# artbataev/end2end

Hardware: AMD Instinct MI355X
Metric: ctc_fwd_bwd_frames_per_sec (higher is better)
Workload: dtype f32; 1 GPU; ctc_fwd_bwd_B256_T1000_V29_S200_f32; B_per_gpu=256, T=1000, V=29, S_max=200, input=raw logits (log-softmax fused)

## Files before the change

### end2end_amd/csrc/ctc_loss_fast_h1.hip

```cpp
#include "fast_common.h"

namespace e2e {
namespace fastk {
namespace {

constexpr int kHxNP = 2;
constexpr int kHxHalo = 8;
constexpr int kHxOwnLanes = 64 - kHxHalo;
constexpr int kHxProducers = 2;
constexpr int kHxOwn = kHxNP * kHxOwnLanes;
constexpr int kHxMaxW = 4 / kHxNP;
constexpr int kHxWaves = 2 * kHxMaxW + 2 + 2 * kHxProducers + 2;

struct HxLds {
  static constexpr int kCkPad = 4;
  static constexpr int kCkCells = 2 * 4 * kHxOwnLanes + 2 * kCkPad;
  int ring;
  int blk_bytes;
  int filled;
  int sortcnt;
  int bnd;
  int bw;
  int dump;
  int zacc;
  int prog;
  int exw;
  int mxl;
  int ckb;
  int ckdone;
  int total;
  __host__ __device__ HxLds(int V) {
    bw = 4;
    ring = 0;
    blk_bytes = ((V + 1) * kRow + 16) * 8;
    filled = ring + 2 * kRingBlks * blk_bytes;
    sortcnt = filled + 2 * kRingBlks * 4;
    bnd = (sortcnt + 130 * 4 + 15) & ~15;
    dump = bnd + 2 * bw * kHaloSlots * kHxHalo * 32;
    zacc = dump + 12288;
    prog = zacc + 64;
    exw = prog + 2 * 8 * 4;
    mxl = exw + 2 * kHaloSlots * 4;
    ckb = mxl + 2 * kHaloSlots * 4 * 64 * 4;
    ckdone = ckb + 2 * 2 * kCkCells * 8;
    total = ckdone + 16;
  }
};

#ifdef E2E_FAST_PROFILE
#define HX_TL(k) { if (w == 0 && lane == 0 && b < 256) { unsigned long long* g = g_tl + ((size_t)b * 2 + DIR) * 12 + 2 * (k); \
    g[0] = __builtin_amdgcn_s_memtime(); g[1] = wall_clock64(); } }
#else
#define HX_TL(k)
#endif
template <int DIR>
__device__ __forceinline__ void hx_chain_wave(const FastParams& p, int b, int T, int S, unsigned char* smem, const HxLds hl,
                                              int lane, int w, int W) {
  lds_u8* L0 = (lds_u8*)smem;
  HX_TL(1)
  const int V = p.V, blank = p.blank, L = 2 * S + 1;
  const int nblk = (T + kBlk - 1) / kBlk;
  const int M = (T - 1) >> 3;
  const int ring_off = hl.ring + DIR * kRingBlks * hl.blk_bytes;
  volatile int* myfilled = reinterpret_cast<int*>(smem + hl.filled) + DIR * kRingBlks;
  __builtin_amdgcn_s_setprio(3);
  unsigned long long prof_fill = 0, prof_nb = 0, prof_lag = 0, prof_t0 = __builtin_amdgcn_s_memtime();
  (void)prof_fill; (void)prof_nb; (void)prof_lag; (void)prof_t0;

  const int g0 = kHxOwn * w + kHxNP * (DIR == 0 ? lane - kHxHalo : lane);
  const bool halo = DIR == 0 ? lane < kHxHalo : lane >= kHxOwnLanes;
  const bool edge = DIR == 0 ? lane >= 64 - kHxHalo : lane < kHxHalo;
  const int up = DIR == 0 ? (w > 0 ? w - 1 : 7) : w + 1;
  const int64_t* tg = p.targets + (int64_t)b * p.tgt_stride;
  const float r_tilt = fast_tilt(S, T);
  const double rr2 = (double)r_tilt * (double)r_tilt, inv_rr = 1.0 / (double)r_tilt;
  const double skip_w = (double)(r_tilt * r_tilt);
  int lab[kHxNP]; double sk[kHxNP];
  bool badlab = false;
#pragma unroll
  for (int r = 0; r < kHxNP; r++) {
    const int gi = g0 + r, li = DIR == 0 ? gi : gi - 1;
    const bool lin = li >= 0 && li < S;
    const int lv = lin ? label_of(tg[li]) : -1;
    lab[r] = (lin && lv >= 0 && lv < V) ? lv : V;
    if (DIR == 0) {
      const int lpv = (li >= 1 && li - 1 < S) ? label_of(tg[li - 1]) : -1;
      sk[r] = (lin && li >= 1 && lv != blank && lpv != lv) ? skip_w : 0.0;
      badlab |= !halo && lin && (lv == blank || lv < 0 || lv >= V);
    } else {
      const int tj = (gi >= 1 && gi < S) ? label_of(tg[gi]) : -1;
      sk[r] = (gi >= 1 && gi < S && lv != blank && tj != lv) ? skip_w : 0.0;
    }
  }
  if (DIR == 0 && __any(badlab)) { if (lane == 0) atomicOr(&p.flags[b], 2); }
  const bool cond = (T > 1 || L == 1);

  const int a_sync = hl.prog;
  const int o_prog = DIR * 32, o_exw = hl.exw - hl.prog + DIR * (kHaloSlots * 4), o_ckdone = hl.ckdone - hl.prog + 4 * DIR;
  const int a_mxl = hl.mxl + ((DIR * kHaloSlots * 4 + w) * 64 + lane) * 4;
  const int up_rec = DIR == 0 ? (w > 0 ? w - 1 : hl.bw - 1) : w + 1;
  const int a_bnd_up = hl.bnd + ((DIR * hl.bw + up_rec) * kHaloSlots * kHxHalo + (lane & (kHxHalo - 1))) * 32;
  const int a_bnd_my = edge ? hl.bnd + ((DIR * hl.bw + w) * kHaloSlots * kHxHalo + (lane & (kHxHalo - 1))) * 32
                            : hl.dump + lane * 32;
  const int a_ck = halo ? hl.dump + 4096 + lane * 32
                        : hl.ckb + (DIR * 2 * HxLds::kCkCells + HxLds::kCkPad) * 8 + (DIR == 0 ? 16 * g0 : 16 * g0 - 8);
  int a_lab[kHxNP];
#pragma unroll
  for (int r = 0; r < kHxNP; r++) a_lab[r] = ring_off + lab[r] * (kRow * 8);
  const int a_yw = ring_off + (V + 1) * (kRow * 8);

  double Bc[kHxNP], Lc[kHxNP];
#pragma unroll
  for (int r = 0; r < kHxNP; r++) { Bc[r] = 0.0; Lc[r] = 0.0; }
  double yb_prev = 0.0, wb_prev = 0.0;
  int e_total = 0;
  int nck = 0, ckbuf = 0;
  int lead = 0;
  auto need_blocks = [&](int k) {
    if (lead < k) {
      PROF_SPIN_BEGIN
      for (;;) {
        int a = peek(&myfilled[0]);
#pragma unroll
        for (int f = 1; f < kHxProducers; f++) a = min(a, peek(&myfilled[f]));
        lead = __builtin_amdgcn_readfirstlane(a);
        if (lead >= k) break;
        __builtin_amdgcn_s_sleep(1);
      }
      asm volatile("" ::: "memory");
      PROF_SPIN_END(prof_fill)
    }
  };

  double e[kHxNP][kBlk], ybw[2 * kBlk];
  auto load_half = [&](int slot_bytes, auto half_tag) {
    constexpr int H = decltype(half_tag)::value;
    lds_u8* py = L0 + (a_yw + slot_bytes);
#pragma unroll
    for (int q = 3; q >= 1; q--) {
      const h_d2 y = *(volatile lds_d2*)(py + 64 * H + 16 * q);
      ybw[8 * H + 2 * q] = y.x; ybw[8 * H + 2 * q + 1] = y.y;
    }
#pragma unroll
    for (int r = 0; r < kHxNP; r++) {
      const h_d2 a = *(volatile lds_d2*)(L0 + (a_lab[r] + slot_bytes) + 32 * H + 16); e[r][4 * H + 2] = a.x; e[r][4 * H + 3] = a.y;
    }
#pragma unroll
    for (int r = 0; r < kHxNP; r++) {
      const h_d2 a = *(volatile lds_d2*)(L0 + (a_lab[r] + slot_bytes) + 32 * H); e[r][4 * H] = a.x; e[r][4 * H + 1] = a.y;
    }
    { const h_d2 y = *(volatile lds_d2*)(py + 64 * H); ybw[8 * H] = y.x; ybw[8 * H + 1] = y.y; }
  };
  auto read_edge = [&](int slot, h_d2 (&hv)[kHxNP]) {
#pragma unroll
    for (int r = 0; r < kHxNP; r++) hv[r] = *(volatile lds_d2*)(L0 + a_bnd_up + slot * 256 + 16 * r);
  };

  int hprog = 0;
  h_d2 hv[kHxNP];
#pragma unroll
  for (int r = 0; r < kHxNP; r++) hv[r] = h_d2{0.0, 0.0};
  int ckd = 0;
  auto run_block = [&](int n, auto steady_tag, auto slot_tag, auto ck_tag) {
    constexpr bool STEADY = decltype(steady_tag)::value;
    constexpr int SLOT = decltype(slot_tag)::value, CK = decltype(ck_tag)::value;
    const int slot = SLOT >= 0 ? SLOT : (n & (kRingBlks - 1));
    const int nslot = SLOT >= 0 ? ((SLOT + 1) & (kRingBlks - 1)) : ((n + 1) & (kRingBlks - 1));
    const int pslot = SLOT >= 0 ? ((SLOT + 7) & (kRingBlks - 1)) : ((n + 7) & (kRingBlks - 1));
    const bool refill = SLOT >= 0 ? (SLOT % kHxNP) == 0 : (n % kHxNP) == 0;
    const bool publish = SLOT >= 0 ? (SLOT % kHxNP) == kHxNP - 1 : (n % kHxNP) == kHxNP - 1;
    load_half(slot * hl.blk_bytes, std::integral_constant<int, 1>{});
    if (refill && (STEADY || n > 0)) {
      if (__builtin_amdgcn_readfirstlane(hprog) < n) {
        PROF_SPIN_BEGIN HALO_WAIT(__builtin_amdgcn_readfirstlane(*(volatile lds_int*)(L0 + a_sync + o_prog + 4 * up)) >= n); PROF_SPIN_END(prof_nb)
        read_edge(pslot, hv);
      }
      if (halo) {
#pragma unroll
        for (int r = 0; r < kHxNP; r++) { Bc[r] = hv[r].x; Lc[r] = hv[r].y; }
      }
    }
    const bool want_next = STEADY ? true : n + 1 < nblk;
    const int tbase = block_time(DIR, n, 0, T);
    int xw = 0;
#pragma unroll
    for (int tt = 0; tt < kBlk; tt++) {
      const int t = DIR == 0 ? tbase + tt : tbase - tt;
      const double yb = ybw[2 * tt], wb = ybw[2 * tt + 1];
      if (tt == 4) {
        xw = *(volatile lds_int*)(L0 + a_sync + o_exw + 4 * slot);
        if (CK != 0) ckd = *(volatile lds_int*)(L0 + a_sync + o_ckdone);
        if (want_next) need_blocks(n + 2);
        load_half(nslot * hl.blk_bytes, std::integral_constant<int, 0>{});
      }
      if (tt == 6 && publish) {
        hprog = *(volatile lds_int*)(L0 + a_sync + o_prog + 4 * up);
        read_edge(slot, hv);
      }
      if (STEADY || t < T) {
        const bool first = !STEADY && (DIR == 0 ? t == 0 : t == T - 1);
        if (first) {
#pragma unroll
          for (int r = 0; r < kHxNP; r++) {
            if (DIR == 0) {
              if (g0 + r == 0) { Bc[r] = cond ? 1.0 : 0.0; Lc[r] = rr2 * e[r][tt]; }
            } else {
              if (g0 + r == S) { if (cond) Bc[r] = 1.0; Lc[r] = rr2 * e[r][tt]; }
            }
          }
        } else if (DIR == 0) {
          double nb = from_prev_lane(Lc[kHxNP - 1]);
#pragma unroll
          for (int r = 0; r < kHxNP; r++) {
            const double ol = Lc[r];
            const double Bn = __builtin_fma(Bc[r], yb_prev, nb);
            double tl = __builtin_fma(Bc[r], wb_prev, ol);
            tl = __builtin_fma(sk[r], nb, tl);
            Lc[r] = tl * e[r][tt]; Bc[r] = Bn; nb = ol;
          }
        } else {
          double nb = from_next_lane(Lc[0]);
#pragma unroll
          for (int r = kHxNP - 1; r >= 0; r--) {
            const double ol = Lc[r];
            const double Bn = __builtin_fma(Bc[r], yb_prev, nb);
            double tl = __builtin_fma(Bc[r], wb_prev, ol);
            tl = __builtin_fma(sk[r], nb, tl);
            Lc[r] = tl * e[r][tt]; Bc[r] = Bn; nb = ol;
          }
        }
        yb_prev = yb; wb_prev = wb;
        if (tt == 7) {
          int top = max(__double2hiint(Bc[0]), __double2hiint(Lc[0]));
#pragma unroll
          for (int r = 1; r < kHxNP; r++) top = max(top, max(__double2hiint(Bc[r]), __double2hiint(Lc[r])));
          *(volatile lds_int*)(L0 + a_mxl + slot * 1024) = top;
          xw = __builtin_amdgcn_readfirstlane(xw);
          if ((xw >> 12) != n) {
            PROF_SPIN_BEGIN
            int spins = 0;
            do {
              __builtin_amdgcn_s_sleep(1);
              xw = __builtin_amdgcn_readfirstlane(*(volatile lds_int*)(L0 + a_sync + o_exw + 4 * slot));
              if (++spins > (1 << 20)) { atomicOr(&p.flags[b], 128); xw = (n << 12) | 2048; }
            } while ((xw >> 12) != n);
            PROF_SPIN_END(prof_lag)
          }
          const int ex = (xw & 0xfff) - 2048;
#pragma unroll
          for (int r = 0; r < kHxNP; r++) { Bc[r] = ldexp(Bc[r], -ex); Lc[r] = ldexp(Lc[r], -ex); }
          e_total += ex;
          const int kk = DIR == 0 ? (t + 1) : t;
          if ((CK >= 0 ? CK == 1 : ((kk & (kSeg - 1)) == 0 && kk > 0 && kk < T))) {
            if (nck >= 2 && __builtin_amdgcn_readfirstlane(ckd) < nck - 1)
              HALO_WAIT(__builtin_amdgcn_readfirstlane(*(volatile lds_int*)(L0 + a_sync + o_ckdone)) >= nck - 1);
            if (nck == 0) ckbuf = (kk / kSeg) & 1;
            nck++;
            lds_u8* dst = L0 + (a_ck + ckbuf * (HxLds::kCkCells * 8));
#pragma unroll
            for (int r = 0; r < kHxNP; r++) {
              const double cb = Bc[r] * yb_prev, cl = Lc[r] * inv_rr;
              if (DIR == 0) { *(volatile lds_f64*)(dst + 16 * r) = cb; *(volatile lds_f64*)(dst + 16 * r + 8) = cl; }
              else { *(volatile lds_f64*)(dst + 16 * r) = cl; *(volatile lds_f64*)(dst + 16 * r + 8) = cb; }
            }
            ckbuf ^= 1;
          }
        }
      }
    }
    if (publish) {
#pragma unroll
      for (int r = 0; r < kHxNP; r++) { h_d2 v; v.x = Bc[r]; v.y = Lc[r]; *(volatile lds_d2*)(L0 + a_bnd_my + slot * 256 + 16 * r) = v; }
    }
    *(volatile lds_int*)(L0 + a_sync + o_prog + 4 * w) = n + 1;
  };
  {
    typedef std::integral_constant<int, -1> Any;
    need_blocks(1);
    HX_TL(2)
    load_half(0, std::integral_constant<int, 0>{});
    const int steady_end = DIR == 0 ? T / kBlk : nblk;
    run_block(0, std::false_type{}, Any{}, Any{});
    int n = 1;
    if (M - 1 >= 16) {
      for (; n < 8; n++) run_block(n, std::true_type{}, Any{}, Any{});
      auto eight = [&](auto par_tag) {
        constexpr int P = decltype(par_tag)::value;
#define HX_BLK(K) run_block(n + K, std::true_type{}, std::integral_constant<int, K>{}, std::integral_constant<int, ((K & 1) == P) ? 1 : 0>{});
        for (; n + 8 <= M; n += 8) { HX_BLK(0) HX_BLK(1) HX_BLK(2) HX_BLK(3) HX_BLK(4) HX_BLK(5) HX_BLK(6) HX_BLK(7) }
#undef HX_BLK
      };
      if (DIR == 0 || (M & 1)) eight(std::integral_constant<int, 1>{});
      else eight(std::integral_constant<int, 0>{});
    }
    for (; n < steady_end - 1; n++) run_block(n, std::true_type{}, Any{}, Any{});
    for (; n < nblk; n++) run_block(n, std::false_type{}, Any{}, Any{});
  }
  HX_TL(3)
#ifdef E2E_FAST_PROFILE
  if (lane == 0 && b < 256) { unsigned long long* g = g_prof3 + ((size_t)b * 16 + DIR * 8 + w) * 4;
    g[0] = __builtin_amdgcn_s_memtime() - prof_t0; g[1] = prof_fill; g[2] = prof_nb; g[3] = prof_lag; }
#endif
  lds_u8* prog = L0 + hl.prog + DIR * 32;
  if (DIR == 0) {
    double z = 0.0;
    if (!halo) {
#pragma unroll
      for (int r = 0; r < kHxNP; r++) {
        if (g0 + r == S) z += Bc[r] * yb_prev;
        if (g0 + r == S - 1) z += Lc[r];
      }
    }
    for (int o = 32; o > 0; o >>= 1) z += __shfl_xor(z, o, 64);
    *(volatile lds_f64*)(L0 + hl.zacc + 8 * w) = z;
    *(volatile lds_int*)(prog + 4 * w) = nblk + 1;
    if (w == 0) {
      HALO_WAIT(__builtin_amdgcn_readfirstlane(lds_min8(prog)) >= nblk + 1);
      if (lane == 0) {
        double zs = 0.0;
        for (int k = 0; k < W; k++) zs += *(volatile lds_f64*)(L0 + hl.zacc + 8 * k);
        const double rr = (double)r_tilt;
        const double lz = log(zs) + (double)e_total * 0.693147180559945309417 - (double)(L - 1) * log(rr);
        p.logz[2 * b] = lz;
        p.zt2[b] = log2(zs) + (double)e_total;
        p.losses[b] = (float)(-lz);
        if (!(zs > 0.0) || !(zs < __builtin_huge_val())) atomicOr(&p.flags[b], 4);
      }
    }
  } else if (w == 0) {
    const double l0 = Lc[kHxNP - 1];
    if (lane == 0) {
      const double z = (cond ? Bc[0] * yb_prev : 0.0) + l0;
      p.logz[2 * b + 1] = log(z) + (double)e_total * 0.693147180559945309417 - (double)(L - 1) * log((double)r_tilt);
    }
  }
  HX_TL(4)
}

template <int NV, int DIR>
__device__ __forceinline__ void hx_prep_wave(const FastParams& p, int b, int T, int first, unsigned char* smem, const HxLds hl,
                                             int lane, double rr2) {
  constexpr int stride = kHxProducers;
  lds_u8* L0 = (lds_u8*)smem;
  const int V = p.V;
  const int nblk = (T + kBlk - 1) / kBlk, M = (T - 1) >> 3;
  const int tt = lane >> 3, l8 = lane & 7;
  const float ninf = -__builtin_huge_valf();
  constexpr int kFull = NV == 2 ? 0 : NV == 12 ? 8 : NV - 2;
  bool live[NV];
#pragma unroll
  for (int k = 0; k < NV; k++) live[k] = k < kFull || l8 + 8 * k < V;
  const bool contig = p.sV == 1;
  const int64_t xl = (int64_t)b * p.sB + (int64_t)l8 * p.sV;
  const int64_t cstep = 8 * p.sV;
  float* yl = p.ytab + ((size_t)b * p.NS * V + l8) * kSeg;
  const int t_first = DIR == 0 ? tt : 8 * M + 7 - tt;
  lds_u8* prog = L0 + hl.prog + DIR * 32;
  const int a_fill = hl.filled + (DIR * kRingBlks + first) * 4;
  const int a_row = hl.ring + DIR * kRingBlks * hl.blk_bytes + (l8 * kRow + tt) * 8;
  const int a_yw = hl.ring + DIR * kRingBlks * hl.blk_bytes + ((V + 1) * kRow + 2 * tt) * 8;
  const int kb = p.blank >> 3;
  const bool blank_lane = l8 == (p.blank & 7);

  auto row_of = [&](int n) { return DIR == 0 ? t_first + 8 * n : t_first - 8 * n; };
  auto load_block = [&](auto f32_tag, int n, float (&out)[NV]) {
    constexpr bool F32IN = decltype(f32_tag)::value;
    const int t = row_of(n);
    const int tc = min(max(t, 0), T - 1);
    const int64_t xr = xl + (int64_t)tc * p.sT;
    int64_t off[NV];
#pragma unroll
    for (int k = 0; k < NV; k++) off[k] = (k < kFull || live[k]) ? (contig ? (int64_t)(8 * k) : k * cstep) : 0;
    if (F32IN) {
      const float* src = reinterpret_cast<const float*>(p.x) + xr;
#pragma unroll
      for (int k = 0; k < NV; k++) out[k] = src[off[k]];
    } else {
      const unsigned short* src = reinterpret_cast<const unsigned short*>(p.x) + xr;
      unsigned short h[NV];
#pragma unroll
      for (int k = 0; k < NV; k++) h[k] = src[off[k]];
      const bool bf = p.xdt == E2E_BF16;
#pragma unroll
      for (int k = 0; k < NV; k++)
        out[k] = bf ? __uint_as_float((unsigned)h[k] << 16) : (float)__builtin_bit_cast(f16_t, h[k]);
    }
  };
  int consumed = 0;
  float lpmin = 0.f;
  auto process = [&](int n, const float (&xraw)[NV]) {
    constexpr bool STEADY = false;
    const int t = row_of(n);
    const bool row_live = t >= 0 && t < T;
    float xv[NV];
#pragma unroll
    for (int k = 0; k < NV; k++) xv[k] = (row_live && (k < kFull || live[k])) ? xraw[k] : ninf;
    if (n >= kRingBlks) {
      while (consumed < n - kRingBlks + 1) {
        consumed = __builtin_amdgcn_readfirstlane(lds_min8(prog));
        if (consumed < n - kRingBlks + 1) __builtin_amdgcn_s_sleep(1);
      }
      asm volatile("" ::: "memory");
    }
    float y[NV];
    if (p.logprobs) {
#pragma unroll
      for (int k = 0; k < NV; k++) {
        y[k] = exp_le0(xv[k]);
        if (DIR == 0) lpmin = fminf(lpmin, xv[k] > ninf ? xv[k] : 0.f);
      }
    } else {
      float m = xv[0];
#pragma unroll
      for (int k = 1; k < NV; k++) m = fmaxf(m, xv[k]);
      m = row8_max(m);
      float ssum = 0.f;
      const float mM = -m * 1.44269504088896340736f;
#pragma unroll
      for (int k = 0; k < NV; k++) {
        const float d = xv[k] - m;
        y[k] = __builtin_amdgcn_exp2f(fmaf(xv[k], 1.44269504088896340736f, mM)); ssum += y[k];
        if (DIR == 0) lpmin = fminf(lpmin, xv[k] > ninf ? d : 0.f);
      }
      ssum = row8_sum(ssum);
      float inv = __builtin_amdgcn_rcpf(ssum);
      inv = fmaf(fmaf(-ssum, inv, 1.0f), inv, inv);
#pragma unroll
      for (int k = 0; k < NV; k++) y[k] *= inv;
    }
    if (!STEADY) {
#pragma unroll
      for (int k = 0; k < NV; k++) y[k] = row_live ? y[k] : 0.f;
    }
    const int sb = (n & (kRingBlks - 1)) * hl.blk_bytes;
    lds_u8* dst = L0 + (a_row + sb);
#pragma unroll
    for (int k = 0; k < NV; k++) {
      if (k < kFull || live[k]) *(volatile lds_f64*)(dst + k * (8 * kRow * 8)) = (double)y[k];
    }
    {
      float ybl = y[0];
#pragma unroll
      for (int k = 1; k < NV; k++) ybl = kb == k ? y[k] : ybl;
      if (blank_lane) { h_d2 yw; yw.x = (double)ybl; yw.y = rr2 * (double)ybl; *(volatile lds_d2*)(L0 + (a_yw + sb)) = yw; }
    }
    if (DIR == 0 && row_live) {
      float* yrow = yl + (size_t)(t >> 4) * V * kSeg + (t & (kSeg - 1));
#pragma unroll
      for (int k = 0; k < NV; k++) {
        if (k < kFull || live[k]) yrow[8 * k * kSeg] = y[k];
      }
    }
    *(volatile lds_int*)(L0 + a_fill) = n + stride;
  };
  auto run = [&](auto f32_tag) {
    float xa[NV], xb[NV], xc[NV];
    load_block(f32_tag, first, xa);
    load_block(f32_tag, first + stride, xb);
    for (int n = first; n < nblk; n += 3 * stride) {
      load_block(f32_tag, n + 2 * stride, xc); process(n, xa);
      load_block(f32_tag, n + 3 * stride, xa); if (n + stride < nblk) process(n + stride, xb);
      load_block(f32_tag, n + 4 * stride, xb); if (n + 2 * stride < nblk) process(n + 2 * stride, xc);
    }
  };
  if (p.xdt == E2E_F32) run(std::true_type{}); else run(std::false_type{});
  { const bool t1 = __any(lpmin < -69.f), t2 = __any(lpmin < -78.f);
    if (DIR == 0 && t1 && lane == 0) atomicOr(&p.flags[b], t2 ? 64 | 256 : 64); }
}

template <int DIR, int F2PPL>
__device__ __forceinline__ void hx_ckpt_wave(const FastParams& p, int b, int T, int S, lds_u8* L0, const HxLds hl, int lane, int npairs) {
  static_assert(F2PPL == 1 || F2PPL == 2 || F2PPL == 4, "groups of up to four lanes (one DPP quad)");
  const int nblk = (T + kBlk - 1) / kBlk;
  const int nres = DIR == 0 ? T / kBlk : nblk;
  const int M = (T - 1) >> 3;
  lds_u8* prog = L0 + hl.prog + DIR * 32;
  float* ck = (DIR == 0 ? p.ckA : p.ckQ) + (size_t)b * p.NS * p.CELLS;
  int done = 0;
  for (int n = 0; n < nres; n++) {
    const int kk = DIR == 0 ? 8 * (n + 1) : 8 * (M - n);
    if (!((kk & (kSeg - 1)) == 0 && kk > 0 && kk < T)) continue;
    HALO_WAIT(__builtin_amdgcn_readfirstlane(lds_min8(prog)) >= n + 1);
    const int slot = kk / kSeg;
    const int base = hl.ckb + ((DIR * 2 + (slot & 1)) * HxLds::kCkCells + HxLds::kCkPad) * 8;
    h_d2 c[4];
#pragma unroll
    for (int q = 0; q < 4; q++) {
      const int i = 64 * q + lane;
      c[q] = h_d2{0.0, 0.0};
      if (64 * q < npairs) c[q] = *(volatile lds_d2*)(L0 + base + 16 * min(i, npairs - 1));
      if (i >= S) c[q].y = 0.0;
      if (i > S) c[q].x = 0.0;
    }
    *(volatile lds_int*)(L0 + hl.ckdone + 4 * DIR) = ++done;
#pragma unroll
    for (int q = 0; q < 4; q++) {
      if (64 * q >= npairs) break;
      const int i = 64 * q + lane;
      int m = max(__double2hiint(c[q].x), __double2hiint(c[q].y));
      if (F2PPL >= 2) m = max(m, dpp_i<0xB1>(0, m));
      if (F2PPL >= 4) m = max(m, dpp_i<0x4E>(0, m));
      const int own = ((m >> 20) & 0x7ff) - 1023;
      const int st = m > 0 ? own : -30000;
      if (i < npairs && (i & ~(F2PPL - 1)) <= S) {
        float2 o;
        o.x = m > 0 ? (float)ldexp(c[q].x, -own) : 0.f; o.y = m > 0 ? (float)ldexp(c[q].y, -own) : 0.f;
        *reinterpret_cast<float2*>(ck + (size_t)slot * p.CELLS + 2 * i) = o;
        short* cke = p.ckE + (((size_t)b * p.NS + slot) * 2 + DIR) * 64;
        if ((i & (F2PPL - 1)) == 0) cke[i / F2PPL] = (short)st;
      }
    }
  }
}

template <int PPL>
__global__ E2E_KERNEL_ALIGN __launch_bounds__(kHxWaves * 64) void ctc_fast_chain_hx_kernel(FastParams p) {
  extern __shared__ __align__(16) unsigned char smem[];
  const int b = blockIdx.x, tid = threadIdx.x, lane = tid & 63, wid = tid >> 6;
  const int V = p.V;
  const HxLds hl(V);
#ifdef E2E_FAST_PROFILE
  if (tid < 128 && lane == 0 && b < 256) { unsigned long long* g = g_tl + ((size_t)b * 2 + (tid >> 6)) * 12; g[0] = __builtin_amdgcn_s_memtime(); g[1] = wall_clock64(); }
#endif

  if (b == 0 && tid < 32) p.ctl[tid] = 0;
  const int64_t Tq = p.x_len[b], Sq = p.t_len[b];
  const bool bad = Tq < 1 || Tq > p.T || Sq < 0 || Sq > p.Smax;
  if (bad) {
    if (tid == 0) { p.flags[b] = 1; p.losses[b] = __builtin_nanf(""); }
    return;
  }
  const int T = (int)Tq, S = (int)Sq;
  const int W = min(S / kHxOwn + 1, kHxMaxW);
  if (tid == 0) p.flags[b] = 0;
  for (int i = tid; i < p.MW; i += blockDim.x) p.segmask[(size_t)b * p.MW + i] = 0u;
  if (tid < 2 * kRingBlks) reinterpret_cast<int*>(smem + hl.filled)[tid] = (tid & (kRingBlks - 1)) < kHxProducers ? (tid & (kRingBlks - 1)) : 0;
  if (tid < 16) reinterpret_cast<int*>(smem + hl.prog)[tid] = (tid & 7) < W ? 0 : kHaloIdle;
  if (tid < 2 * kHaloSlots) reinterpret_cast<int*>(smem + hl.exw)[tid] = (tid & (kHaloSlots - 1)) < kHaloLag ? ((tid & (kHaloSlots - 1)) << 12) | 2048 : -1;
  if (tid < 8) reinterpret_cast<double*>(smem + hl.zacc)[tid] = 0.0;
  if (tid < 2) reinterpret_cast<int*>(smem + hl.ckdone)[tid] = 0;
  for (int i = tid; i < (hl.dump - hl.bnd) / 16; i += blockDim.x) reinterpret_cast<double2*>(smem + hl.bnd)[i] = double2{0.0, 0.0};
  for (int i = tid; i < 2 * kRingBlks * kBlk; i += blockDim.x)
    reinterpret_cast<double*>(smem + hl.ring + (i / kBlk) * hl.blk_bytes)[V * kRow + (i % kBlk)] = 0;
  __syncthreads();

  constexpr int kChains = 2 * kHxMaxW, kFrame = kChains, kProd = kChains + 2, kCkpt = kProd + 2 * kHxProducers;
  const int wave = __builtin_amdgcn_readfirstlane(wid);
  lds_u8* L0 = (lds_u8*)smem;
  if (wave < kChains) {
    const int d = wave & 1, w = wave >> 1;
    if (w >= W) return;
    if (d == 0) hx_chain_wave<0>(p, b, T, S, smem, hl, lane, w, W);
    else hx_chain_wave<1>(p, b, T, S, smem, hl, lane, w, W);
  } else if (wave == kFrame) halo_frame_wave<0, false, kHaloLag, true>(p, b, T, L0, hl.prog, hl.exw, hl.mxl, 4, lane, W, 0);
  else if (wave == kFrame + 1) halo_frame_wave<1, false, kHaloLag, true>(p, b, T, L0, hl.prog, hl.exw, hl.mxl, 4, lane, W, 0);
  else if (wave == kCkpt) hx_ckpt_wave<0, PPL>(p, b, T, S, L0, hl, lane, kHxOwn * W);
  else if (wave == kCkpt + 1) {
    cellinfo_wave<PPL>(p, b, T, S, reinterpret_cast<int*>(smem + hl.sortcnt), lane);
    hx_ckpt_wave<1, PPL>(p, b, T, S, L0, hl, lane, kHxOwn * W);
  } else {
    const int d = (wave - kProd) & 1;
    const int first = (wave - kProd) >> 1;
    const double rr2 = (double)fast_tilt(S, T) * (double)fast_tilt(S, T);
#define HX_PREP(NVV) { if (d == 0) hx_prep_wave<NVV, 0>(p, b, T, first, smem, hl, lane, rr2); else hx_prep_wave<NVV, 1>(p, b, T, first, smem, hl, lane, rr2); }
    if (V <= 16) HX_PREP(2) else if (V <= 32) HX_PREP(4) else if (V <= 48) HX_PREP(6) else if (V <= 64) HX_PREP(8) else HX_PREP(12)
#undef HX_PREP
  }
}

}

bool h1_supported(int V, int Smax, int ppl) {
  return (ppl == 2 || ppl == 4) && Smax + 1 <= 4 * kHxOwnLanes && HxLds(V).total <= 160 * 1024;
}

Chains h1_chains(int ppl, int V) {
  return Chains{ppl == 4 ? &ctc_fast_chain_hx_kernel<4> : &ctc_fast_chain_hx_kernel<2>, kHxWaves * 64, (size_t)HxLds(V).total};
}

}
}

#ifdef E2E_FAST_PROFILE
extern "C" int e2e_debug_fast_timeline_h1(unsigned long long* host) {
  return hipMemcpyFromSymbol(host, HIP_SYMBOL(e2e::fastk::g_tl), sizeof(unsigned long long) * 256 * 2 * 12) == hipSuccess ? 0 : E2E_ERR_HIP;
}
extern "C" int e2e_debug_fast_profile3_h1(unsigned long long* host, int reset) {
  if (reset) { void* ptr; if (hipGetSymbolAddress(&ptr, HIP_SYMBOL(e2e::fastk::g_prof3)) != hipSuccess) return E2E_ERR_HIP;
    return hipMemset(ptr, 0, sizeof(unsigned long long) * 256 * 16 * 4) == hipSuccess ? 0 : E2E_ERR_HIP; }
  return hipMemcpyFromSymbol(host, HIP_SYMBOL(e2e::fastk::g_prof3), sizeof(unsigned long long) * 256 * 16 * 4) == hipSuccess ? 0 : E2E_ERR_HIP;
}
#endif
```

### end2end_amd/csrc/fast_common.h

```cpp
#pragma once
#include <stdlib.h>
#include <type_traits>

#include "common.h"

#pragma clang fp contract(fast)

#define E2E_KERNEL_ALIGN __attribute__((aligned(65536)))

namespace e2e {
namespace fastk {

constexpr int kSeg = kFastSeg;
constexpr int kBlk = 8;
constexpr int kRingBlks = 8;
constexpr int kRow32 = 12;
constexpr int kRow = 10;
constexpr int kMaxSmallV = 96;
constexpr int kMaxBigV = 224;
constexpr int kMaxHugeV = 448;
__host__ __device__ inline int lstart_ints(int V) { return 64 * ((V + 64) >> 6) + 2; }

struct FastParams {
  const void* x; int xdt;
// ... 73 lines not shown
  v += __int_as_float(__builtin_amdgcn_update_dpp(0, __float_as_int(v), 0x111, 0xf, 0xf, true));
  v += __int_as_float(__builtin_amdgcn_update_dpp(0, __float_as_int(v), 0x112, 0xf, 0xf, true));
  v += __int_as_float(__builtin_amdgcn_update_dpp(0, __float_as_int(v), 0x114, 0xf, 0xf, true));
  v += __int_as_float(__builtin_amdgcn_update_dpp(0, __float_as_int(v), 0x118, 0xf, 0xf, true));
  E2E_ROW_BCAST_STEPS("v_add_f32_dpp", v);
  return v;
}
__device__ __forceinline__ void wave_scan8(float (&v)[8]) {
#pragma unroll
  for (int k = 0; k < 8; k++) v[k] += __int_as_float(__builtin_amdgcn_update_dpp(0, __float_as_int(v[k]), 0x111, 0xf, 0xf, true));
#pragma unroll
  for (int k = 0; k < 8; k++) v[k] += __int_as_float(__builtin_amdgcn_update_dpp(0, __float_as_int(v[k]), 0x112, 0xf, 0xf, true));
#pragma unroll
  for (int k = 0; k < 8; k++) v[k] += __int_as_float(__builtin_amdgcn_update_dpp(0, __float_as_int(v[k]), 0x114, 0xf, 0xf, true));
#pragma unroll
  for (int k = 0; k < 8; k++) v[k] += __int_as_float(__builtin_amdgcn_update_dpp(0, __float_as_int(v[k]), 0x118, 0xf, 0xf, true));
  asm volatile("s_nop 1\n\t"
               "v_add_f32_dpp %0, %0, %0 row_bcast:15 row_mask:0xa bank_mask:0xf\n\t"
               "v_add_f32_dpp %1, %1, %1 row_bcast:15 row_mask:0xa bank_mask:0xf\n\t"
               "v_add_f32_dpp %2, %2, %2 row_bcast:15 row_mask:0xa bank_mask:0xf\n\t"
               "v_add_f32_dpp %3, %3, %3 row_bcast:15 row_mask:0xa bank_mask:0xf\n\t"
               "v_add_f32_dpp %4, %4, %4 row_bcast:15 row_mask:0xa bank_mask:0xf\n\t"
               "v_add_f32_dpp %5, %5, %5 row_bcast:15 row_mask:0xa bank_mask:0xf\n\t"
               "v_add_f32_dpp %6, %6, %6 row_bcast:15 row_mask:0xa bank_mask:0xf\n\t"
               "v_add_f32_dpp %7, %7, %7 row_bcast:15 row_mask:0xa bank_mask:0xf\n\t"
               "v_add_f32_dpp %0, %0, %0 row_bcast:31 row_mask:0xc bank_mask:0xf\n\t"
               "v_add_f32_dpp %1, %1, %1 row_bcast:31 row_mask:0xc bank_mask:0xf\n\t"
               "v_add_f32_dpp %2, %2, %2 row_bcast:31 row_mask:0xc bank_mask:0xf\n\t"
               "v_add_f32_dpp %3, %3, %3 row_bcast:31 row_mask:0xc bank_mask:0xf\n\t"
               "v_add_f32_dpp %4, %4, %4 row_bcast:31 row_mask:0xc bank_mask:0xf\n\t"
               "v_add_f32_dpp %5, %5, %5 row_bcast:31 row_mask:0xc bank_mask:0xf\n\t"
               "v_add_f32_dpp %6, %6, %6 row_bcast:31 row_mask:0xc bank_mask:0xf\n\t"
               "v_add_f32_dpp %7, %7, %7 row_bcast:31 row_mask:0xc bank_mask:0xf"
               : "+v"(v[0]), "+v"(v[1]), "+v"(v[2]), "+v"(v[3]), "+v"(v[4]), "+v"(v[5]), "+v"(v[6]), "+v"(v[7]));
}
__device__ __forceinline__ int wave_scan(int v) {
  v += __builtin_amdgcn_update_dpp(0, v, 0x111, 0xf, 0xf, true);
  v += __builtin_amdgcn_update_dpp(0, v, 0x112, 0xf, 0xf, true);
  v += __builtin_amdgcn_update_dpp(0, v, 0x114, 0xf, 0xf, true);
  v += __builtin_amdgcn_update_dpp(0, v, 0x118, 0xf, 0xf, true);
  E2E_ROW_BCAST_STEPS("v_add_u32_dpp", v);
  return v;
}
__device__ __forceinline__ int wave_scan_max(int v) {
  v = max(v, __builtin_amdgcn_update_dpp(v, v, 0x111, 0xf, 0xf, false));
  v = max(v, __builtin_amdgcn_update_dpp(v, v, 0x112, 0xf, 0xf, false));
  v = max(v, __builtin_amdgcn_update_dpp(v, v, 0x114, 0xf, 0xf, false));
  v = max(v, __builtin_amdgcn_update_dpp(v, v, 0x118, 0xf, 0xf, false));
  E2E_ROW_BCAST_STEPS("v_max_i32_dpp", v);
  return v;
}

__device__ __forceinline__ void wave_sum8(const float (&v)[8], float (&tot)[8], int lane) {
  const bool b0 = lane & 1, b1 = lane & 2;
  float w[4], u[2];
#pragma unroll
  for (int j = 0; j < 4; j++) {
    const float keep = b0 ? v[j + 4] : v[j], send = b0 ? v[j] : v[j + 4];
    w[j] = keep + __int_as_float(dpp_i<0xB1>(0, __float_as_int(send)));
  }
#pragma unroll
  for (int j = 0; j < 2; j++) {
    const float keep = b1 ? w[j + 2] : w[j], send = b1 ? w[j] : w[j + 2];
    u[j] = keep + __int_as_float(dpp_i<0x4E>(0, __float_as_int(send)));
  }
#pragma unroll
  for (int j = 0; j < 2; j++) {
    u[j] += __int_as_float(dpp_i<0x124>(0, __float_as_int(u[j])));
    u[j] += __int_as_float(dpp_i<0x128>(0, __float_as_int(u[j])));
  }
#pragma unroll
  for (int j = 0; j < 2; j++) u[j] += __shfl_xor(u[j], 16, 64);
#pragma unroll
  for (int j = 0; j < 2; j++) u[j] += __shfl_xor(u[j], 32, 64);
#pragma unroll
  for (int c = 0; c < 4; c++) {
    const int row = 4 * (c & 1) + 2 * (c >> 1);
    tot[row] = __int_as_float(__builtin_amdgcn_readlane(__float_as_int(u[0]), c));
    tot[row + 1] = __int_as_float(__builtin_amdgcn_readlane(__float_as_int(u[1]), c));
  }
}

__device__ __forceinline__ float row16_max(float v) {
  v = fmaxf(v, __int_as_float(dpp_i<0xB1>(0, __float_as_int(v))));
  v = fmaxf(v, __int_as_float(dpp_i<0x4E>(0, __float_as_int(v))));
  v = fmaxf(v, __int_as_float(dpp_i<0x141>(0, __float_as_int(v))));
  v = fmaxf(v, __int_as_float(dpp_i<0x140>(0, __float_as_int(v))));
  return v;
}
__device__ __forceinline__ float row16_sum(float v) {
  v += __int_as_float(dpp_i<0xB1>(0, __float_as_int(v)));
  v += __int_as_float(dpp_i<0x4E>(0, __float_as_int(v)));
  v += __int_as_float(dpp_i<0x141>(0, __float_as_int(v)));
  v += __int_as_float(dpp_i<0x140>(0, __float_as_int(v)));
  return v;
}

__device__ __forceinline__ float row8_max(float v) {
  v = fmaxf(v, __int_as_float(dpp_i<0xB1>(0, __float_as_int(v))));
  v = fmaxf(v, __int_as_float(dpp_i<0x4E>(0, __float_as_int(v))));
  v = fmaxf(v, __int_as_float(dpp_i<0x141>(0, __float_as_int(v))));
  return v;
}
__device__ __forceinline__ float row8_sum(float v) {
  v += __int_as_float(dpp_i<0xB1>(0, __float_as_int(v)));
  v += __int_as_float(dpp_i<0x4E>(0, __float_as_int(v)));
  v += __int_as_float(dpp_i<0x141>(0, __float_as_int(v)));
  return v;
}

#ifdef E2E_FAST_PROFILE
static __device__ unsigned long long g_prof[256 * 4 * 4];
static __device__ unsigned long long g_prof2[16384 * 8];
static __device__ unsigned long long g_prof3[256 * 16 * 4];
static __device__ float g_zdev[16384];
static __device__ unsigned long long g_tl[256 * 2 * 12];
__shared__ unsigned long long s_prof_prev;
__shared__ unsigned long long s_prof_acc[8];
#define F2_STAMP(i) { unsigned long long _t; asm volatile("s_waitcnt vmcnt(0) lgkmcnt(0)\n s_memtime %0\n s_waitcnt lgkmcnt(0)" : "=s"(_t) :: "memory"); \
    if (threadIdx.x == 0) { if ((i) < 0) { for (int _k = 0; _k < 8; _k++) s_prof_acc[_k] = 0; } else s_prof_acc[(i) < 0 ? 0 : (i)] += _t - s_prof_prev; } \
    asm volatile("s_waitcnt lgkmcnt(0)\n s_memtime %0\n s_waitcnt lgkmcnt(0)" : "=s"(_t) :: "memory"); if (threadIdx.x == 0) s_prof_prev = _t; asm volatile("s_waitcnt lgkmcnt(0)" ::: "memory"); }
#define F2_FLUSH { const unsigned _wg = blockIdx.y * gridDim.x + blockIdx.x; if (threadIdx.x < 8 && _wg < 16384) g_prof2[_wg * 8 + threadIdx.x] = s_prof_acc[threadIdx.x]; }
#define PROF_SPIN_BEGIN unsigned long long _t0 = __builtin_amdgcn_s_memtime();
#define PROF_SPIN_END(acc) acc += __builtin_amdgcn_s_memtime() - _t0;
#else
#define PROF_SPIN_BEGIN
#define PROF_SPIN_END(acc)
#define F2_STAMP(i)
#define F2_FLUSH
#endif
__host__ __device__ inline size_t align_up_dev(size_t x, size_t a) { return (x + a - 1) / a * a; }
typedef __attribute__((address_space(3))) int lds_int;
__device__ __forceinline__ void spin_until(volatile int* p, int want) {
  volatile lds_int* q = (volatile lds_int*)p;
  while (*q != want) __builtin_amdgcn_s_sleep(1);
  asm volatile("" ::: "memory");
}
__device__ __forceinline__ void spin_until_ge(volatile int* p, int want) {
  volatile lds_int* q = (volatile lds_int*)p;
  while (*q < want) __builtin_amdgcn_s_sleep(1);
  asm volatile("" ::: "memory");
}
__device__ __forceinline__ void publish(volatile int* p, int v) {
  asm volatile("" ::: "memory");
  *(volatile lds_int*)p = v;
}
__device__ __forceinline__ int peek(volatile int* p) { return *(volatile lds_int*)p; }
typedef __attribute__((address_space(3))) unsigned char lds_u8;
typedef double h_d2 __attribute__((ext_vector_type(2)));
typedef int h_i4 __attribute__((ext_vector_type(4)));
typedef __attribute__((address_space(3))) h_d2 lds_d2;
typedef __attribute__((address_space(3))) double lds_f64;
typedef __attribute__((address_space(3))) h_i4 lds_i4;

__device__ __forceinline__ int lds_min8(lds_u8* a) {
  const h_i4 u = *(volatile lds_i4*)a, v = *(volatile lds_i4*)(a + 16);
  return min(min(min(u.x, u.y), min(u.z, u.w)), min(min(v.x, v.y), min(v.z, v.w)));
}
__device__ __forceinline__ int lds_max8(lds_u8* a) {
  const h_i4 u = *(volatile lds_i4*)a, v = *(volatile lds_i4*)(a + 16);
  return max(max(max(u.x, u.y), max(u.z, u.w)), max(max(v.x, v.y), max(v.z, v.w)));
}

template <int PPL>
struct LaneCells {
  int lab[PPL];
  float skp[PPL];
  float skn[PPL];
  float r;
  bool has_blank_label;
  __device__ void set_tilt(int S, int T) {
    r = fast_tilt(S, T);
  }
  __device__ static unsigned pack(int lab, int slot, float skp, float skn) {
    return (unsigned)lab | ((unsigned)slot << 10) | (skp != 0.f ? 1u << 20 : 0u) | (skn != 0.f ? 1u << 21 : 0u);
  }
  __device__ void unpack(const unsigned* w, int S, int T, int (&slot)[PPL]) {
    set_tilt(S, T);
    has_blank_label = false;
#pragma unroll
    for (int q = 0; q < PPL; q++) {
      lab[q] = (int)(w[q] & 0x3ffu);
      slot[q] = (int)((w[q] >> 10) & 0x3ffu);
      skp[q] = (w[q] >> 20) & 1u ? r * r : 0.f;
      skn[q] = (w[q] >> 21) & 1u ? r * r : 0.f;
    }
  }
  __device__ void load(const int64_t* tg, int S, int T, int V, int blank, int lane) {
    has_blank_label = false;
    set_tilt(S, T);
#pragma unroll
    for (int q = 0; q < PPL; q++) {
      const int i = PPL * lane + q;
      const int li = i < S ? label_of(tg[i]) : -1;
      const int lp = (i >= 1 && i - 1 < S) ? label_of(tg[i - 1]) : -1;
      const int ln = (i + 1 < S) ? label_of(tg[i + 1]) : -1;
      lab[q] = i < S ? li : V;
      skp[q] = (i < S && i >= 1 && li != blank && lp != li) ? r * r : 0.f;
      skn[q] = (i + 1 < S && li != blank && ln != li) ? r * r : 0.f;
      if (i < S && (li == blank || li < 0 || li >= V)) has_blank_label = true;
      if (i < S && (li < 0 || li >= V)) lab[q] = V;
    }
  }
};

struct F1Lds {
  double* ring;
  int* filled;
  int* took;
  int* sortcnt;
  int blk_elems;
  static constexpr int kSyncInts = 2 * kRingBlks + 2;
  __device__ F1Lds(unsigned char* smem, int V, int rb = kRingBlks) {
    blk_elems = (V + 1) * kRow;
    ring = reinterpret_cast<double*>(smem);
    filled = reinterpret_cast<int*>(ring + 2 * rb * blk_elems);
    took = filled + 2 * kRingBlks;
    sortcnt = took + 2;
  }
  __host__ __device__ static size_t bytes(int V, int rb = kRingBlks) { return sizeof(double) * 2 * rb * (V + 1) * kRow + sizeof(int) * (kSyncInts + 130); }
};

__device__ __forceinline__ int block_time(int dir, int n, int tt, int T) {
  return dir == 0 ? n * kBlk + tt : (((T - 1) >> 3) - n) * kBlk + 7 - tt;
}

__device__ __forceinline__ float exp_le0(float x) {
  x = fmaxf(x, -200.f);
  const float t = x * 1.44269504088896340736f;
  const float n = rintf(t);
  float f = fmaf(x, 1.44269504088896340736f, -n);
  f = fmaf(x, 1.92596299112661746e-8f, f);
  return ldexpf(__builtin_amdgcn_exp2f(f), (int)n);
}

template <int NV, int MODE = 0, int RB = kRingBlks>
__device__ __forceinline__ void prep_wave(const FastParams& p, int b, int T, int dir, int first, int stride,
                                          unsigned char* myring_bytes, int blk_bytes, volatile int* myfilled, volatile int* took,
                                          int lane, lds_u8* prog = nullptr, double rr2 = 0.0) {
  constexpr bool HALO = MODE != 0;
  const int V = p.V;
  const int nblk = (T + kBlk - 1) / kBlk;
  const int64_t xo = (int64_t)b * p.sB;
  float* ytab = p.ytab + (size_t)b * p.NS * kSeg * V;
  const int tt = lane >> 3, l8 = lane & 7;
  const float ninf = -__builtin_huge_valf();
  bool col_live[NV];
  int64_t col_off[NV];
#pragma unroll
  for (int k = 0; k < NV; k++) { col_live[k] = l8 + 8 * k < V; col_off[k] = (int64_t)(col_live[k] ? l8 + 8 * k : 0) * p.sV; }
  unsigned long long prof_spin = 0, prof_t0 = __builtin_amdgcn_s_memtime();
  (void)prof_spin; (void)prof_t0;
  auto load_block = [&](auto f32_tag, int n, float (&out)[NV]) {
    constexpr bool F32IN = decltype(f32_tag)::value;
    const int t = block_time(dir, n, tt, T);
    const bool row_live = n < nblk && t < T;
    const int64_t xr = xo + (int64_t)(row_live ? t : 0) * p.sT;
    if (F32IN) {
#pragma unroll
      for (int k = 0; k < NV; k++) out[k] = reinterpret_cast<const float*>(p.x)[xr + col_off[k]];
    } else {
      unsigned short h[NV];
#pragma unroll
      for (int k = 0; k < NV; k++) h[k] = reinterpret_cast<const unsigned short*>(p.x)[xr + col_off[k]];
      const bool bf = p.xdt == E2E_BF16;
#pragma unroll
      for (int k = 0; k < NV; k++)
        out[k] = bf ? __uint_as_float((unsigned)h[k] << 16) : (float)__builtin_bit_cast(f16_t, h[k]);
    }
  };
  int consumed = 0;
  float lpmin = 0.f;
  auto process = [&](int n, const float (&xraw)[NV]) {
    if (n >= nblk) return;
    float xv[NV];
    {
      const bool row_in = block_time(dir, n, tt, T) < T;
#pragma unroll
      for (int k = 0; k < NV; k++) xv[k] = (row_in && col_live[k]) ? xraw[k] : ninf;
    }
    const int slot = n % RB;
    if (n >= RB) {
      PROF_SPIN_BEGIN
      if (HALO) {
        while (consumed < n - RB + 1) {
          consumed = __builtin_amdgcn_readfirstlane(lds_min8(prog));
          if (consumed < n - RB + 1) __builtin_amdgcn_s_sleep(1);
        }
        asm volatile("" ::: "memory");
      } else spin_until_ge(took, n - RB + 1);
      PROF_SPIN_END(prof_spin)
    }
    double* blk = reinterpret_cast<double*>(myring_bytes + (size_t)slot * blk_bytes);
    float* blk32 = reinterpret_cast<float*>(myring_bytes + (size_t)slot * blk_bytes);
    const int t = block_time(dir, n, tt, T);
    const bool row_live = t < T;
    float y[NV];
    if (p.logprobs) {
#pragma unroll
      for (int k = 0; k < NV; k++) {
        y[k] = exp_le0(xv[k]);
        lpmin = fminf(lpmin, xv[k] > ninf ? xv[k] : 0.f);
      }
    } else {
      float m = xv[0];
#pragma unroll
// ... 214 lines not shown
```

Measured before the change: 2.378 billion frames/s.

## Relayout LDS with constexpr offsets, separate blank-yw ring, early fill prefetch

Turns the LDS layout offsets into compile-time constants. It moves the sync words to offset 0 and pulls the blank/yw values out of the per-block ring into their own small array, so address arithmetic folds into immediate offsets. It also prefetches the two producers' fill counters as one 8-byte load two timesteps early, so the consumer spin usually skips a separate LDS round trip. The checkpoint store becomes a single 16-byte write with a simpler double-buffer offset toggle. The risks are extra register pressure from the early loads and changed timing in the producer/consumer handshake.

```diff
diff --git a/end2end_amd/csrc/ctc_loss_fast_h1.hip b/end2end_amd/csrc/ctc_loss_fast_h1.hip
--- a/end2end_amd/csrc/ctc_loss_fast_h1.hip
+++ b/end2end_amd/csrc/ctc_loss_fast_h1.hip
@@ -15,35 +15,25 @@
 struct HxLds {
   static constexpr int kCkPad = 4;
   static constexpr int kCkCells = 2 * 4 * kHxOwnLanes + 2 * kCkPad;
-  int ring;
+  static constexpr int bw = 4;
+  static constexpr int prog = 0;
+  static constexpr int exw = prog + 2 * 8 * 4;
+  static constexpr int filled = exw + 2 * kHaloSlots * 4;
+  static constexpr int ckdone = filled + 2 * kRingBlks * 4;
+  static constexpr int zacc = ckdone + 16;
+  static constexpr int sortcnt = zacc + 64;
+  static constexpr int yw = (sortcnt + 130 * 4 + 15) & ~15;
+  static constexpr int bnd = yw + 2 * kRingBlks * 128;
+  static constexpr int dump = bnd + 2 * bw * kHaloSlots * kHxHalo * 32;
+  static constexpr int mxl = dump + 12288;
+  static constexpr int ckb = mxl + 2 * kHaloSlots * 4 * 64 * 4;
+  static constexpr int ring = ckb + 2 * 2 * kCkCells * 8;
+  static_assert(filled % 8 == 0 && yw % 16 == 0 && bnd % 16 == 0 && dump % 16 == 0 && ckb % 16 == 0 && ring % 16 == 0, "alignment of the wide accesses");
   int blk_bytes;
-  int filled;
-  int sortcnt;
-  int bnd;
-  int bw;
-  int dump;
-  int zacc;
-  int prog;
-  int exw;
-  int mxl;
-  int ckb;
-  int ckdone;
   int total;
   __host__ __device__ HxLds(int V) {
-    bw = 4;
-    ring = 0;
-    blk_bytes = ((V + 1) * kRow + 16) * 8;
-    filled = ring + 2 * kRingBlks * blk_bytes;
-    sortcnt = filled + 2 * kRingBlks * 4;
-    bnd = (sortcnt + 130 * 4 + 15) & ~15;
-    dump = bnd + 2 * bw * kHaloSlots * kHxHalo * 32;
-    zacc = dump + 12288;
-    prog = zacc + 64;
-    exw = prog + 2 * 8 * 4;
-    mxl = exw + 2 * kHaloSlots * 4;
-    ckb = mxl + 2 * kHaloSlots * 4 * 64 * 4;
-    ckdone = ckb + 2 * 2 * kCkCells * 8;
-    total = ckdone + 16;
+    blk_bytes = (V + 1) * kRow * 8;
+    total = ring + 2 * kRingBlks * blk_bytes;
   }
 };
 
@@ -95,8 +85,12 @@
   if (DIR == 0 && __any(badlab)) { if (lane == 0) atomicOr(&p.flags[b], 2); }
   const bool cond = (T > 1 || L == 1);
 
-  const int a_sync = hl.prog;
+  int vz;
+  asm volatile("v_mov_b32 %0, 0" : "=v"(vz));
+  const int a_sync = vz + hl.prog;
   const int o_prog = DIR * 32, o_exw = hl.exw - hl.prog + DIR * (kHaloSlots * 4), o_ckdone = hl.ckdone - hl.prog + 4 * DIR;
+  const int o_filled = hl.filled - hl.prog + DIR * (kRingBlks * 4);
+  const int a_up = a_sync + o_prog + 4 * up, a_me = a_sync + o_prog + 4 * w;
   const int a_mxl = hl.mxl + ((DIR * kHaloSlots * 4 + w) * 64 + lane) * 4;
   const int up_rec = DIR == 0 ? (w > 0 ? w - 1 : hl.bw - 1) : w + 1;
   const int a_bnd_up = hl.bnd + ((DIR * hl.bw + up_rec) * kHaloSlots * kHxHalo + (lane & (kHxHalo - 1))) * 32;
@@ -107,16 +101,18 @@
   int a_lab[kHxNP];
 #pragma unroll
   for (int r = 0; r < kHxNP; r++) a_lab[r] = ring_off + lab[r] * (kRow * 8);
-  const int a_yw = ring_off + (V + 1) * (kRow * 8);
+  const int a_yw = vz + hl.yw + DIR * (kRingBlks * 128);
 
   double Bc[kHxNP], Lc[kHxNP];
 #pragma unroll
   for (int r = 0; r < kHxNP; r++) { Bc[r] = 0.0; Lc[r] = 0.0; }
   double yb_prev = 0.0, wb_prev = 0.0;
   int e_total = 0;
-  int nck = 0, ckbuf = 0;
+  int nck = 0, ckoff = (DIR == 0 ? 1 : (M >> 1) & 1) * (HxLds::kCkCells * 8);
   int lead = 0;
-  auto need_blocks = [&](int k) {
+  static_assert(kHxProducers == 2, "the early look reads the two producers' words as one 8-byte pair");
+  auto need_blocks = [&](int k, h_i2 early) {
+    if (lead < k) lead = __builtin_amdgcn_readfirstlane(min(early.x, early.y));
     if (lead < k) {
       PROF_SPIN_BEGIN
       for (;;) {
@@ -133,9 +129,10 @@
   };
 
   double e[kHxNP][kBlk], ybw[2 * kBlk];
-  auto load_half = [&](int slot_bytes, auto half_tag) {
+  auto load_half = [&](int slot, auto half_tag) {
     constexpr int H = decltype(half_tag)::value;
-    lds_u8* py = L0 + (a_yw + slot_bytes);
+    const int slot_bytes = slot * hl.blk_bytes;
+    lds_u8* py = L0 + (a_yw + slot * 128);
 #pragma unroll
     for (int q = 3; q >= 1; q--) {
       const h_d2 y = *(volatile lds_d2*)(py + 64 * H + 16 * q);
@@ -169,10 +166,10 @@
     const int pslot = SLOT >= 0 ? ((SLOT + 7) & (kRingBlks - 1)) : ((n + 7) & (kRingBlks - 1));
     const bool refill = SLOT >= 0 ? (SLOT % kHxNP) == 0 : (n % kHxNP) == 0;
     const bool publish = SLOT >= 0 ? (SLOT % kHxNP) == kHxNP - 1 : (n % kHxNP) == kHxNP - 1;
-    load_half(slot * hl.blk_bytes, std::integral_constant<int, 1>{});
+    load_half(slot, std::integral_constant<int, 1>{});
     if (refill && (STEADY || n > 0)) {
       if (__builtin_amdgcn_readfirstlane(hprog) < n) {
-        PROF_SPIN_BEGIN HALO_WAIT(__builtin_amdgcn_readfirstlane(*(volatile lds_int*)(L0 + a_sync + o_prog + 4 * up)) >= n); PROF_SPIN_END(prof_nb)
+        PROF_SPIN_BEGIN HALO_WAIT(__builtin_amdgcn_readfirstlane(*(volatile lds_int*)(L0 + a_up)) >= n); PROF_SPIN_END(prof_nb)
         read_edge(pslot, hv);
       }
       if (halo) {
@@ -183,18 +180,23 @@
     const bool want_next = STEADY ? true : n + 1 < nblk;
     const int tbase = block_time(DIR, n, 0, T);
     int xw = 0;
+    h_i2 fill2 = h_i2{0, 0};
 #pragma unroll
     for (int tt = 0; tt < kBlk; tt++) {
       const int t = DIR == 0 ? tbase + tt : tbase - tt;
       const double yb = ybw[2 * tt], wb = ybw[2 * tt + 1];
+      if (tt == 2 && want_next) {
+        fill2 = *(volatile lds_i2*)(L0 + a_sync + o_filled);
+        __builtin_amdgcn_sched_barrier(0);
+      }
       if (tt == 4) {
         xw = *(volatile lds_int*)(L0 + a_sync + o_exw + 4 * slot);
         if (CK != 0) ckd = *(volatile lds_int*)(L0 + a_sync + o_ckdone);
-        if (want_next) need_blocks(n + 2);
-        load_half(nslot * hl.blk_bytes, std::integral_constant<int, 0>{});
+        if (want_next) need_blocks(n + 2, fill2);
+        load_half(nslot, std::integral_constant<int, 0>{});
       }
       if (tt == 6 && publish) {
-        hprog = *(volatile lds_int*)(L0 + a_sync + o_prog + 4 * up);
+        hprog = *(volatile lds_int*)(L0 + a_up);
         read_edge(slot, hv);
       }
       if (STEADY || t < T) {
@@ -252,18 +254,17 @@
           e_total += ex;
           const int kk = DIR == 0 ? (t + 1) : t;
           if ((CK >= 0 ? CK == 1 : ((kk & (kSeg - 1)) == 0 && kk > 0 && kk < T))) {
-            if (nck >= 2 && __builtin_amdgcn_readfirstlane(ckd) < nck - 1)
+            if (__builtin_amdgcn_readfirstlane(ckd) < nck - 1)
               HALO_WAIT(__builtin_amdgcn_readfirstlane(*(volatile lds_int*)(L0 + a_sync + o_ckdone)) >= nck - 1);
-            if (nck == 0) ckbuf = (kk / kSeg) & 1;
             nck++;
-            lds_u8* dst = L0 + (a_ck + ckbuf * (HxLds::kCkCells * 8));
+            lds_u8* dst = L0 + (a_ck + ckoff);
 #pragma unroll
             for (int r = 0; r < kHxNP; r++) {
               const double cb = Bc[r] * yb_prev, cl = Lc[r] * inv_rr;
-              if (DIR == 0) { *(volatile lds_f64*)(dst + 16 * r) = cb; *(volatile lds_f64*)(dst + 16 * r + 8) = cl; }
-              else { *(volatile lds_f64*)(dst + 16 * r) = cl; *(volatile lds_f64*)(dst + 16 * r + 8) = cb; }
+              if (DIR == 0) { h_d2 c; c.x = cb; c.y = cl; *(volatile lds_d2*)(dst + 16 * r) = c; }
+              else { h_d2 c; c.x = cl; c.y = cb; *(volatile lds_d2_a8*)(dst + 16 * r) = c; }
             }
-            ckbuf ^= 1;
+            ckoff ^= HxLds::kCkCells * 8;
           }
         }
       }
@@ -272,11 +273,11 @@
 #pragma unroll
       for (int r = 0; r < kHxNP; r++) { h_d2 v; v.x = Bc[r]; v.y = Lc[r]; *(volatile lds_d2*)(L0 + a_bnd_my + slot * 256 + 16 * r) = v; }
     }
-    *(volatile lds_int*)(L0 + a_sync + o_prog + 4 * w) = n + 1;
+    *(volatile lds_int*)(L0 + a_me) = n + 1;
   };
   {
     typedef std::integral_constant<int, -1> Any;
-    need_blocks(1);
+    need_blocks(1, h_i2{0, 0});
     HX_TL(2)
     load_half(0, std::integral_constant<int, 0>{});
     const int steady_end = DIR == 0 ? T / kBlk : nblk;
@@ -358,7 +359,7 @@
   lds_u8* prog = L0 + hl.prog + DIR * 32;
   const int a_fill = hl.filled + (DIR * kRingBlks + first) * 4;
   const int a_row = hl.ring + DIR * kRingBlks * hl.blk_bytes + (l8 * kRow + tt) * 8;
-  const int a_yw = hl.ring + DIR * kRingBlks * hl.blk_bytes + ((V + 1) * kRow + 2 * tt) * 8;
+  const int a_yw = hl.yw + DIR * (kRingBlks * 128) + 2 * tt * 8;
   const int kb = p.blank >> 3;
   const bool blank_lane = l8 == (p.blank & 7);
 
@@ -442,7 +443,7 @@
       float ybl = y[0];
 #pragma unroll
       for (int k = 1; k < NV; k++) ybl = kb == k ? y[k] : ybl;
-      if (blank_lane) { h_d2 yw; yw.x = (double)ybl; yw.y = rr2 * (double)ybl; *(volatile lds_d2*)(L0 + (a_yw + sb)) = yw; }
+      if (blank_lane) { h_d2 yw; yw.x = (double)ybl; yw.y = rr2 * (double)ybl; *(volatile lds_d2*)(L0 + (a_yw + (n & (kRingBlks - 1)) * 128)) = yw; }
     }
     if (DIR == 0 && row_live) {
       float* yrow = yl + (size_t)(t >> 4) * V * kSeg + (t & (kSeg - 1));
diff --git a/end2end_amd/csrc/fast_common.h b/end2end_amd/csrc/fast_common.h
--- a/end2end_amd/csrc/fast_common.h
+++ b/end2end_amd/csrc/fast_common.h
@@ -249,6 +249,9 @@
 typedef __attribute__((address_space(3))) h_d2 lds_d2;
 typedef __attribute__((address_space(3))) double lds_f64;
 typedef __attribute__((address_space(3))) h_i4 lds_i4;
+typedef int h_i2 __attribute__((ext_vector_type(2)));
+typedef __attribute__((address_space(3))) h_i2 lds_i2;
+typedef __attribute__((address_space(3), aligned(8))) h_d2 lds_d2_a8;
 
 __device__ __forceinline__ int lds_min8(lds_u8* a) {
   const h_i4 u = *(volatile lds_i4*)a, v = *(volatile lds_i4*)(a + 16);
```

Result: faster. 2.443 billion frames/s (median of 6 runs) (+2.7%).
